# secondmind-labs/trieste

Hardware: NVIDIA H100
Metric: acquisition candidate-points/sec (EI on GPR N=4096 fp64) (higher is better)
Workload: dtype f64

## Files before the change

### trieste_b200/csrc/prescreen.cuh

```cuda
#pragma once
#include <cuda_fp16.h>
#include "kernels_f64.cuh"

namespace tb {
namespace pre {

constexpr int KS = 64;
constexpr int KH = 32;
constexpr int TH = 256;
template <int DP> struct Cpt { static constexpr int value = DP <= 12 ? 4 : DP <= 20 ? 2 : 1; };
template <int DP> struct Row { static constexpr int W = ((DP + 3 + 3) / 4) * 4; };

__host__ __device__ constexpr int tc_nk(int dp) { return (3 * dp + 2 + 15) / 16; }
__host__ __device__ constexpr int tc_mt(int dp) { return tc_nk(dp) <= 2 ? 4 : tc_nk(dp) <= 4 ? 2 : 1; }
__host__ __device__ constexpr int tc_slices(int dp) { return tc_nk(dp) <= 2 ? 16 : 8; }
__host__ __device__ constexpr int tc_slice_bytes(int dp) { return 256 * tc_nk(dp) + 32; }
__host__ __device__ constexpr int tc_cands(int dp) { return 16 * tc_mt(dp) * (TH / 32); }

struct Bound {
  double rel;
  double lin;
  double lin_max;
  double abs;
  double safety;
  double x2max;
  double mean_const;
  double pre;
};

__device__ __forceinline__ float ex2_approx(float x) {
  float y;
  asm("ex2.approx.ftz.f32 %0, %1;" : "=f"(y) : "f"(x));
  return y;
}
__device__ __forceinline__ float rsqrt_approx(float x) {
  float y;
  asm("rsqrt.approx.ftz.f32 %0, %1;" : "=f"(y) : "f"(x));
  return y;
}

template <int KIND>
__device__ __forceinline__ float kfun(float q) {
  constexpr float LN2 = 0.693147180559945309f, LN2SQ3 = 0.160151031252949358f;
  if (KIND == TB_RBF) return ex2_approx(-q);
  q = fmaxf(q, 1e-30f);
  const float s = q * rsqrt_approx(q);
  const float e = ex2_approx(-s);
  if (KIND == TB_MATERN12) return e;
  if (KIND == TB_MATERN32) return fmaf(s, LN2, 1.0f) * e;
  return fmaf(q, LN2SQ3, fmaf(s, LN2, 1.0f)) * e;
}

__device__ __forceinline__ void bound_out(const Bound& b, int64_t t, double lg, double mu, double s, int acq, double param,
                                          double var_ub, double* __restrict__ out0, double* __restrict__ out1, double& bv,
                                          int64_t& bi) {
  double e = b.safety * (fma(b.rel + lg, s, b.abs));
  const double mt = b.mean_const + mu;
  if (!(lg <= b.lin_max) || !(e <= DBL_MAX)) e = NAN;
  if (acq < 0) {
    out0[t] = mt - e;
    out1[t] = mt + e;
  } else {
    out0[t] = acq_value(acq, param, 0.0, mt - e, var_ub);
    const double v = acq_value(acq, param, 0.0, mt, var_ub);
    if (v == v) best_merge(bv, bi, v, t);
  }
}

template <int KIND, int DP>
__global__ void __launch_bounds__(TH, 2)
mean_bounds_kernel(const float* __restrict__ rows, int nst, const double* __restrict__ Xc, const double* __restrict__ inv_ls,
                   const double* __restrict__ centre, int D, int64_t M, const __grid_constant__ Bound b, int acq, double param,
                   double var_ub, double* __restrict__ out0, double* __restrict__ out1, double* __restrict__ blk_best,
                   int64_t* __restrict__ blk_idx) {
  constexpr int CPT = Cpt<DP>::value, W = Row<DP>::W, CH = KS * W / 4;
  constexpr bool EXPAND = KIND != TB_MATERN12;
  __shared__ __align__(16) float rs[2][KS * W];
  const int64_t t0 = (int64_t)blockIdx.x * (TH * CPT) + threadIdx.x;
  float xc[CPT][DP], xc2[CPT];
#pragma unroll
  for (int c = 0; c < CPT; ++c) {
    const int64_t t = t0 + (int64_t)c * TH;
    xc2[c] = 0.0f;
#pragma unroll
    for (int d = 0; d < DP; ++d) {
      xc[c][d] = (t < M && d < D) ? (float)((Xc[t * D + d] * inv_ls[d] - centre[d]) * b.pre) : 0.0f;
      xc2[c] = fmaf(xc[c][d], xc[c][d], xc2[c]);
    }
  }
  auto stage_load = [&](int kc, int buf) {
    const float* src = rows + (int64_t)kc * KS * W;
#pragma unroll
    for (int i = 0; i < (CH + TH - 1) / TH; ++i) {
      const int e = i * TH + (int)threadIdx.x;
      if (e < CH) asm volatile("cp.async.cg.shared.global [%0], [%1], 16;" ::"r"(smem_u32(&rs[buf][4 * e])), "l"(src + 4 * e) : "memory");
    }
    asm volatile("cp.async.commit_group;" ::: "memory");
  };
  double mu_d[CPT], s_d[CPT];
#pragma unroll
  for (int c = 0; c < CPT; ++c) mu_d[c] = s_d[c] = 0.0;
  stage_load(0, 0);
  for (int kc = 0; kc < nst; ++kc) {
    const int buf = kc & 1;
    if (kc + 1 < nst) {
      stage_load(kc + 1, buf ^ 1);
      asm volatile("cp.async.wait_group 1;" ::: "memory");
    } else {
      asm volatile("cp.async.wait_group 0;" ::: "memory");
    }
    __syncthreads();
#pragma unroll
    for (int h = 0; h < KS / KH; ++h) {
      float mu[CPT], sa[CPT];
#pragma unroll
      for (int c = 0; c < CPT; ++c) mu[c] = sa[c] = 0.0f;
#pragma unroll 4
      for (int j = h * KH; j < (h + 1) * KH; ++j) {
        float xr[W];
#pragma unroll
        for (int i = 0; i < W; i += 4) {
          const float4 v = *reinterpret_cast<const float4*>(&rs[buf][j * W + i]);
          xr[i] = v.x, xr[i + 1] = v.y, xr[i + 2] = v.z, xr[i + 3] = v.w;
        }
#pragma unroll
        for (int c = 0; c < CPT; ++c) {
          float q;
          if (EXPAND) {
            float dot = 0.0f;
#pragma unroll
            for (int d = 0; d < DP; ++d) dot = fmaf(xc[c][d], xr[d], dot);
            q = fmaf(-2.0f, dot, xc2[c] + xr[DP]);
          } else {
            q = 0.0f;
#pragma unroll
            for (int d = 0; d < DP; ++d) {
              const float df = xc[c][d] - xr[d];
              q = fmaf(df, df, q);
            }
          }
          const float f = kfun<KIND>(q);
          mu[c] = fmaf(xr[DP + 1], f, mu[c]);
          sa[c] = fmaf(xr[DP + 2], f, sa[c]);
        }
      }
#pragma unroll
      for (int c = 0; c < CPT; ++c) {
        mu_d[c] += (double)mu[c];
        s_d[c] += (double)sa[c];
      }
    }
    __syncthreads();
  }
  double bv = -INFINITY;
  int64_t bi = INT64_MAX;
#pragma unroll
  for (int c = 0; c < CPT; ++c) {
    const int64_t t = t0 + (int64_t)c * TH;
    if (t >= M) continue;
    const double x2 = (double)xc2[c];
    const double lg = EXPAND ? b.lin * (x2 + b.x2max) : b.lin * (sqrt(x2) + sqrt(b.x2max));
    bound_out(b, t, lg, mu_d[c], s_d[c], acq, param, var_ub, out0, out1, bv, bi);
  }
  if (acq >= 0) block_best_store(bv, bi, blk_best, blk_idx);
}

__device__ __forceinline__ void mma_f16(float (&c)[4], const uint32_t (&a)[4], uint32_t b0, uint32_t b1) {
  asm("mma.sync.aligned.m16n8k16.row.col.f32.f16.f16.f32 {%0,%1,%2,%3}, {%4,%5,%6,%7}, {%8,%9}, {%0,%1,%2,%3};"
      : "+f"(c[0]), "+f"(c[1]), "+f"(c[2]), "+f"(c[3])
      : "r"(a[0]), "r"(a[1]), "r"(a[2]), "r"(a[3]), "r"(b0), "r"(b1));
}

template <int KIND, int DP>
__global__ void __launch_bounds__(TH, 2)
tc_mean_bounds_kernel(const unsigned char* __restrict__ cols, int nsl, int npos_sl, const double* __restrict__ Xc,
                      const double* __restrict__ inv_ls, const double* __restrict__ centre, int D, int64_t M,
                      const __grid_constant__ Bound b, int acq, double param, double var_ub, double* __restrict__ out0,
                      double* __restrict__ out1, double* __restrict__ blk_best, int64_t* __restrict__ blk_idx) {
  constexpr int NK = tc_nk(DP), K = 16 * NK, MT = tc_mt(DP), SL = tc_slices(DP), SLB = tc_slice_bytes(DP);
  constexpr int CB = tc_cands(DP), STB = SL * SLB;
  constexpr int CAND_BYTES = CB * (2 * K + 4), SMEM = CAND_BYTES > 2 * STB ? CAND_BYTES : 2 * STB;
  static_assert(KIND != TB_MATERN12 && STB % 16 == 0 && SMEM <= 48 * 1024, "tc_mean_bounds_kernel geometry");
  __shared__ __align__(16) unsigned char sm[SMEM];
  const int64_t c0 = (int64_t)blockIdx.x * CB;
  {
    __half* sa = reinterpret_cast<__half*>(sm);
    float* sx2 = reinterpret_cast<float*>(sm + CB * 2 * K);
    for (int c = threadIdx.x; c < CB; c += TH) {
      const int64_t t = c0 + c;
      __half* row = sa + c * K;
      float x2 = 0.0f;
#pragma unroll
      for (int d = 0; d < DP; ++d) {
        const float x = (t < M && d < D) ? (float)((Xc[t * D + d] * inv_ls[d] - centre[d]) * b.pre) : 0.0f;
        x2 = fmaf(x, x, x2);
        const __half hi = __float2half_rn(x);
        row[d] = row[2 * DP + d] = hi;
        row[DP + d] = __float2half_rn(x - __half2float(hi));
      }
      row[3 * DP] = row[3 * DP + 1] = __float2half_rn(1.0f);
#pragma unroll
      for (int k = 3 * DP + 2; k < K; ++k) row[k] = __float2half_rn(0.0f);
      sx2[c] = x2;
    }
  }
  __syncthreads();
  const int warp = threadIdx.x >> 5, lane = threadIdx.x & 31, g = lane >> 2, tg = lane & 3;
  uint32_t af[MT][NK][4];
  float cx[MT][2];
#pragma unroll
  for (int m = 0; m < MT; ++m) {
    const int r = (warp * MT + m) * 16 + g;
    const __half* sa = reinterpret_cast<const __half*>(sm);
#pragma unroll
    for (int kk = 0; kk < NK; ++kk) {
      const __half* p = sa + r * K + kk * 16 + 2 * tg;
      af[m][kk][0] = *reinterpret_cast<const uint32_t*>(p);
      af[m][kk][1] = *reinterpret_cast<const uint32_t*>(p + 8 * K);
      af[m][kk][2] = *reinterpret_cast<const uint32_t*>(p + 8);
      af[m][kk][3] = *reinterpret_cast<const uint32_t*>(p + 8 * K + 8);
    }
    const float* sx2 = reinterpret_cast<const float*>(sm + CB * 2 * K);
    cx[m][0] = sx2[r];
    cx[m][1] = sx2[r + 8];
  }
  __syncthreads();

  auto stage_load = [&](int kc, int buf) {
    const unsigned char* src = cols + (int64_t)kc * STB;
#pragma unroll
    for (int i = 0; i < (STB / 16 + TH - 1) / TH; ++i) {
      const int e = i * TH + (int)threadIdx.x;
      if (e < STB / 16) asm volatile("cp.async.cg.shared.global [%0], [%1], 16;" ::"r"(smem_u32(sm + buf * STB + 16 * e)), "l"(src + 16 * e) : "memory");
    }
    asm volatile("cp.async.commit_group;" ::: "memory");
  };
  auto slice = [&](const unsigned char* sp, float (&acc)[MT][2]) {
    uint32_t bf[NK][2];
    if constexpr (NK % 2 == 0) {
#pragma unroll
      for (int kk = 0; kk < NK; kk += 2) {
        const uint4 v = reinterpret_cast<const uint4*>(sp)[(lane * NK + kk) / 2];
        bf[kk][0] = v.x, bf[kk][1] = v.y, bf[kk + 1][0] = v.z, bf[kk + 1][1] = v.w;
      }
    } else {
#pragma unroll
      for (int kk = 0; kk < NK; ++kk) {
        const uint2 v = reinterpret_cast<const uint2*>(sp)[lane * NK + kk];
        bf[kk][0] = v.x, bf[kk][1] = v.y;
      }
    }
    const float2 w = reinterpret_cast<const float2*>(sp + 256 * NK)[tg];
#pragma unroll
    for (int m = 0; m < MT; ++m) {
      float c[4] = {cx[m][0], cx[m][0], cx[m][1], cx[m][1]};
#pragma unroll
      for (int kk = 0; kk < NK; ++kk) mma_f16(c, af[m][kk], bf[kk][0], bf[kk][1]);
#pragma unroll
      for (int i = 0; i < 4; ++i) {
        acc[m][i >> 1] = fmaf(i & 1 ? w.y : w.x, kfun<KIND>(c[i]), acc[m][i >> 1]);
      }
    }
  };

  double pd[MT][2], qd[MT][2];
#pragma unroll
  for (int m = 0; m < MT; ++m) pd[m][0] = pd[m][1] = qd[m][0] = qd[m][1] = 0.0;
  const int nst = (nsl + SL - 1) / SL;
  stage_load(0, 0);
  for (int kc = 0; kc < nst; ++kc) {
    const int buf = kc & 1;
    if (kc + 1 < nst) {
      stage_load(kc + 1, buf ^ 1);
      asm volatile("cp.async.wait_group 1;" ::: "memory");
    } else {
      asm volatile("cp.async.wait_group 0;" ::: "memory");
    }
    __syncthreads();
    const unsigned char* st = sm + buf * STB;
    const int s0 = kc * SL, pe = min(SL, nsl - s0), bnd = min(max(npos_sl - s0, 0), pe);
    auto run = [&](int sa, int sb, double (&dd)[MT][2]) {
      float acc[MT][2];
#pragma unroll
      for (int m = 0; m < MT; ++m) acc[m][0] = acc[m][1] = 0.0f;
#pragma unroll 1
      for (int s = sa; s < sb; ++s) slice(st + s * SLB, acc);
#pragma unroll
      for (int m = 0; m < MT; ++m) dd[m][0] += (double)acc[m][0], dd[m][1] += (double)acc[m][1];
    };
    run(0, bnd, pd);
    run(bnd, pe, qd);
    __syncthreads();
  }
  double bv = -INFINITY;
  int64_t bi = INT64_MAX;
#pragma unroll
  for (int m = 0; m < MT; ++m)
#pragma unroll
    for (int h = 0; h < 2; ++h) {
      pd[m][h] += __shfl_xor_sync(0xffffffffu, pd[m][h], 1);
      qd[m][h] += __shfl_xor_sync(0xffffffffu, qd[m][h], 1);
      pd[m][h] += __shfl_xor_sync(0xffffffffu, pd[m][h], 2);
      qd[m][h] += __shfl_xor_sync(0xffffffffu, qd[m][h], 2);
      const int64_t t = c0 + (warp * MT + m) * 16 + g + 8 * h;
      if ((2 * m + h) % 4 != tg || t >= M) continue;
      const double x2 = (double)cx[m][h];
      const double lg = x2 < 0x1p28 ? b.lin * (x2 + b.x2max) : NAN;
      bound_out(b, t, lg, pd[m][h] - qd[m][h], pd[m][h] + qd[m][h], acq, param, var_ub, out0, out1, bv, bi);
    }
  if (acq >= 0) block_best_store(bv, bi, blk_best, blk_idx);
}

__global__ void probe_kernel(const double* __restrict__ Xc, int D, const int64_t* __restrict__ probe, double* __restrict__ xsel,
                             int64_t* __restrict__ isel) {
  int64_t p = *probe;
  if (p == INT64_MAX) p = 0;
  for (int d = threadIdx.x; d < D; d += blockDim.x) xsel[d] = Xc[p * D + d];
  if (threadIdx.x == 0) isel[0] = p;
}

__global__ void __launch_bounds__(256)
compact_kernel(const double* __restrict__ Xc, const double* __restrict__ ub, int64_t M, int64_t split, int D, double var_ub,
               int acq, const double* __restrict__ run_best, int64_t cap, unsigned long long* __restrict__ count,
               double* __restrict__ xsel, int64_t* __restrict__ isel) {
  const int64_t t = (int64_t)blockIdx.x * blockDim.x + threadIdx.x;
  const double thr = screen_threshold(acq, *run_best, var_ub);
  const bool keep = t < M && !(ub[t] < thr);
  const bool back = t >= split;
  const unsigned ball = __ballot_sync(0xffffffffu, keep);
  if (ball == 0u) return;
  const int lane = threadIdx.x & 31;
  const unsigned bb = __ballot_sync(0xffffffffu, keep && back), bf = ball & ~bb;
  unsigned long long base_f = 0, base_b = 0;
  if (lane == 0) {
    if (bf) base_f = atomicAdd(&count[0], (unsigned long long)__popc(bf));
    if (bb) base_b = atomicAdd(&count[1], (unsigned long long)__popc(bb));
  }
  base_f = __shfl_sync(0xffffffffu, base_f, 0);
  base_b = __shfl_sync(0xffffffffu, base_b, 0);
  if (!keep) return;
  const unsigned below = (1u << lane) - 1u;
  const int64_t r = back ? (int64_t)(base_b + (unsigned long long)__popc(bb & below)) : (int64_t)(base_f + (unsigned long long)__popc(bf & below));
  if (r >= cap) return;
  const int64_t pos = back ? cap - 1 - r : r;
  for (int d = 0; d < D; ++d) xsel[pos * D + d] = Xc[t * D + d];
  isel[pos] = t;
}

}
}
```

### trieste_b200/csrc/tb_api.cu

```cuda
#include "gp_handle.cuh"
#include "kernels_extra.cuh"
#include "prescreen.cuh"
#include "batch_ei.cuh"
#include "ehvi.cuh"
#include "int8_engines.h"
#include <chrono>
#include "factor.cuh"
#include "lbfgs.cuh"

using namespace tb;
namespace tb {
int kernels_init();
}

namespace tb {

__global__ void scale_inputs_kernel(const double* __restrict__ X, const double* __restrict__ inv_ls,
                                    int64_t N, int D, int DP, int64_t rows, double* __restrict__ Xs) {
  int64_t i = (int64_t)blockIdx.x * blockDim.x + threadIdx.x;
  if (i >= rows * DP) return;
  int64_t k = i / DP;
  int d = (int)(i % DP);
  Xs[i] = (k < N && d < D) ? X[k * D + d] * inv_ls[d] : 0.0;
}
// ... 587 lines not shown
  gp->nkc = (int)((N + BK - 1) / BK);
  gp->NB = (int)((N + BM - 1) / BM);
  gp->cache_valid = false;
  const int64_t rows = (int64_t)gp->NB * BM;
  TB_TRY(scale_inputs(gp));
  TB_TRY(gp->dAlpha.reserve(sizeof(double) * rows));
  TB_TRY(gp->sA.reserve(sizeof(double) * (3 * cap_rows * APPEND_MAX + 2 * APPEND_MAX * APPEND_MAX)));
  double* W = gp->sA.as<double>();
  double* Y = W + N * m;
  double* U = Y + N * m;
  double* S = U + N * m;
  double* R = S + m * m;
  TB_TRY(gp->dInfo.reserve(sizeof(int)));
  TB_CUDA(cudaMemsetAsync(gp->dInfo.p, 0, sizeof(int), st));
  {
    dim3 grid((unsigned)((N + 127) / 128), (unsigned)m);
    const double* Xs = gp->dXs.as<double>();
    with_kind(gp->kernel, [&](auto K) {
      append_cross_kernel<decltype(K)::value><<<grid, 128, 0, st>>>(Xs, DP, N0, N, gp->variance, gp->noise, W);
    });
    TB_LAUNCHED();
  }
  double* L = gp->dL.as<double>();
  double* Linv = gp->dLinv.as<double>();
  trmv_lower_cols_kernel<<<dim3((unsigned)((N0 + 127) / 128), (unsigned)m), 128, 0, st>>>(Linv, N0, N, W, N, Y, N);
  TB_LAUNCHED();
  append_schur_kernel<<<dim3((unsigned)m, (unsigned)m), 256, 0, st>>>(Y, W, N0, N, (int)m, S);
  TB_LAUNCHED();
  append_chol_kernel<<<1, APPEND_MAX, 0, st>>>(S, (int)m, N0, N, L, Linv, R, gp->dInfo.as<int>());
  TB_LAUNCHED();
  trmv_lower_t_cols_kernel<<<dim3((unsigned)((N0 + 7) / 8), (unsigned)m), 256, 0, st>>>(Linv, N0, N, Y, N, U, N);
  TB_LAUNCHED();
  append_rows_kernel<<<dim3((unsigned)((N0 + 127) / 128), (unsigned)m), 128, 0, st>>>(Y, U, R, (int)m, N0, N, L, Linv);
  TB_LAUNCHED();
  int info = 0;
  TB_CUDA(cudaMemcpyAsync(&info, gp->dInfo.p, sizeof(int), cudaMemcpyDeviceToHost, st));
  TB_CUDA(cudaStreamSynchronize(st));
  TB_CUDA(cudaGetLastError());
  TB_CHECK_CODE(info == 0, "tb_gp_append_data: Cholesky decomposition was not successful "
                      "(K + noise*I not positive definite at leading minor " + std::to_string(info) + ")", tb::ERR_NUMERIC);
  TB_TRY(alpha_from_linv(gp));
  return finish_cache(gp, N0);
}

int tb_gp_get_cholesky(tb_gp* gp, void* L_user) {
  TB_CHECK(gp && L_user, "tb_gp_get_cholesky: null argument");
  TB_CHECK(gp->cache_valid, "tb_gp_get_cholesky: posterior cache is not built");
  const int64_t N = gp->N;
  tb::DtypeBridge br(gp);
  double* L_out;
  TB_TRY(br.out(L_user, N * N, &L_out));
  TB_CUDA(cudaSetDevice(gp->device));
  TB_TRY(gp->sMisc.reserve(sizeof(double) * N * N));
  dim3 grid((unsigned)((N + 127) / 128), (unsigned)N);
  colmajor_lower_to_rowmajor_kernel<<<grid, 128, 0, gp->stream>>>(gp->dL.as<double>(), N, gp->sMisc.as<double>());
  TB_LAUNCHED();
  TB_CUDA(cudaMemcpyAsync(L_out, gp->sMisc.p, sizeof(double) * N * N, cudaMemcpyDefault, gp->stream));
  TB_CUDA(cudaStreamSynchronize(gp->stream));
  return br.finish();
}

}

namespace tb {

struct EvalRequest {
  int acq = -1;
  double param = 0.0;
  const double* Xc = nullptr;
  int64_t M = 0;
  double* out_vals = nullptr;
  double* out_mean = nullptr;
  double* out_var = nullptr;
  double* out_grad = nullptr;
  bool want_argmax = false;
  bool pen = false;
  double best_value = 0.0;
  int64_t best_index = -1;
};

static int launch_kstar(tb_gp* gp, const double* Xc_dev, int64_t mc, int tiles, double* KsP, double* mean) {
  const double* Xs = gp->dXs.as<double>();
  const double* al = gp->dAlpha.as<double>();
  const double* il = gp->dInvLs.as<double>();
  const int N = (int)gp->N, nkc = gp->nkc, D = gp->D;
  const double var = gp->variance, mc0 = gp->mean_const;
  cudaStream_t st = gp->stream;
  with_kind_dp(gp->kernel, gp->DP, [&](auto K, auto P) {
    kstar_panels_kernel<decltype(K)::value, decltype(P)::value><<<tiles, 512, 0, st>>>(Xs, al, Xc_dev, il, N, nkc, D, mc, 0, var, mc0,
                                                                                        KsP, mean);
  });
  TB_LAUNCHED();
  TB_CUDA(cudaGetLastError());
  return 0;
}

static int64_t chunk_tiles(const tb_gp* gp) {
  const size_t per_tile = (size_t)gp->nkc * PANEL * sizeof(double);
  const size_t budget = (size_t)1536 << 20;
  int64_t t = (int64_t)(budget / per_tile);
  t = std::max<int64_t>(t, 1);
  if (t >= NUM_SMS) t = (t / NUM_SMS) * NUM_SMS;
  return std::min<int64_t>(t, NUM_SMS * 16);
}

int kernels_init() {
  TB_CUDA(cudaFuncSetAttribute(fac::chol_diag_kernel, cudaFuncAttributeMaxDynamicSharedMemorySize, (int)(sizeof(double) * fac::FB * (fac::FB + 1))));
  TB_CUDA(cudaFuncSetAttribute(fac::chol_panel_kernel, cudaFuncAttributeMaxDynamicSharedMemorySize, (int)fac::GEMM_SMEM));
  TB_CUDA(cudaFuncSetAttribute(fac::chol_syrk_kernel, cudaFuncAttributeMaxDynamicSharedMemorySize, (int)fac::GEMM_SMEM));
  TB_CUDA(cudaFuncSetAttribute(fac::trinv_level_kernel<1>, cudaFuncAttributeMaxDynamicSharedMemorySize, (int)fac::GEMM_SMEM));
  TB_CUDA(cudaFuncSetAttribute(fac::trinv_level_kernel<2>, cudaFuncAttributeMaxDynamicSharedMemorySize, (int)fac::GEMM_SMEM));
  TB_CUDA(cudaFuncSetAttribute(fac::kinv_kernel, cudaFuncAttributeMaxDynamicSharedMemorySize, (int)fac::GEMM_SMEM));
  TB_TRY(int8_init());
  TB_CUDA(cudaFuncSetAttribute(trigemm_kernel<false, EPI_SUMSQ>, cudaFuncAttributeMaxDynamicSharedMemorySize, (int)TG_SMEM));
  TB_CUDA(cudaFuncSetAttribute(trigemm_kernel<false, EPI_SUMSQ_PACKED>, cudaFuncAttributeMaxDynamicSharedMemorySize, (int)TG_SMEM));
  TB_CUDA(cudaFuncSetAttribute(trigemm_kernel<false, EPI_PLAIN>, cudaFuncAttributeMaxDynamicSharedMemorySize, (int)TG_SMEM));
  TB_CUDA(cudaFuncSetAttribute(trigemm_kernel<true, EPI_PLAIN>, cudaFuncAttributeMaxDynamicSharedMemorySize, (int)TG_SMEM));
  return 0;
}

static int ensure_upper_panels(tb_gp* gp) {
  if (gp->upper_gen == gp->cache_gen) return 0;
  const int nkB = gp->NB * (BM / BK);
  const int64_t np = upper_panel_count(gp->NB, nkB);
  TB_TRY(gp->dLinvTP.reserve(sizeof(double) * np * PANEL));
  dim3 grid((unsigned)nkB, (unsigned)gp->NB);
  pack_upper_panels_kernel<<<grid, 256, 0, gp->stream>>>(gp->dLinv.as<double>(), gp->N, gp->NB, nkB,
                                                         gp->dLinvTP.as<double>());
  TB_LAUNCHED();
  TB_CUDA(cudaGetLastError());
  gp->upper_gen = gp->cache_gen;
  return 0;
}

static int launch_grad(tb_gp* gp, const double* xc, int64_t mc, double* grad_dev) {
  const bool wide = mc <= 2048;
  const int blocks = wide ? (int)mc : (int)((mc + 7) / 8);
  const double* Xs = gp->dXs.as<double>();
  const double* al = gp->dAlpha.as<double>();
  const double* il = gp->dInvLs.as<double>();
  const double* V = gp->sV.as<double>();
  const int64_t ldv = (int64_t)gp->NB * BM;
  const double* cmu = gp->sMisc.as<double>();
  const double* cvar = cmu + mc;
  with_kind_dp(gp->kernel, gp->DP, [&](auto K, auto P) {
    constexpr int KIND = decltype(K)::value, DP = decltype(P)::value;
    if (wide)
      grad_kernel<KIND, DP, 8><<<blocks, 256, 0, gp->stream>>>(Xs, al, xc, il, (int)gp->N, gp->D, mc, V, ldv, cmu, cvar, gp->variance,
                                                               fm::Consts(), grad_dev);
    else
      grad_kernel<KIND, DP, 1><<<blocks, 256, 0, gp->stream>>>(Xs, al, xc, il, (int)gp->N, gp->D, mc, V, ldv, cmu, cvar, gp->variance,
                                                               fm::Consts(), grad_dev);
  });
  TB_LAUNCHED();
  TB_CUDA(cudaGetLastError());
  return 0;
}

static inline bool gibbon_repulsion_kind(int acq) { return acq == TB_ACQ_GIBBON_REPULSION || acq == TB_ACQ_GIBBON; }

static int launch_gibbon_cross(tb_gp* gp, cudaStream_t st, const double* xc, int64_t mc, bool keep_u) {
  TB_TRY(gp->sGib.reserve(sizeof(double) * (size_t)mc * (2 + (keep_u ? gp->gibMp : 0))));
  double* uu = gp->sGib.as<double>();
  double* U = keep_u ? uu + 2 * mc : nullptr;
  const unsigned blocks = (unsigned)((mc + 127) / 128);
  with_kind_dp(gp->kernel, gp->DP, [&](auto K, auto P) {
    gibbon_cross_kernel<decltype(K)::value, decltype(P)::value><<<blocks, 128, 0, st>>>(
        gp->dXs.as<double>(), gp->dGibWhat.as<double>(), gp->dGibPs.as<double>(), gp->dGibLinv.as<double>(), xc, gp->dInvLs.as<double>(),
        (int)gp->N, gp->D, gp->gibM, gp->gibMp, mc, gp->variance, fm::Consts(), uu, U);
  });
  TB_LAUNCHED();
  TB_CUDA(cudaGetLastError());
  return 0;
}

static int launch_gibbon_grad(tb_gp* gp, cudaStream_t st, const double* xc, int64_t mc, double* gd) {
  const double* uu = gp->sGib.as<double>();
  const unsigned blocks = (unsigned)((mc + 7) / 8);
  with_kind_dp(gp->kernel, gp->DP, [&](auto K, auto P) {
    gibbon_grad_kernel<decltype(K)::value, decltype(P)::value><<<blocks, 256, 0, st>>>(
        gp->dXs.as<double>(), gp->dGibWhat.as<double>(), gp->dGibPs.as<double>(), gp->dGibLinv.as<double>(), xc, gp->dInvLs.as<double>(),
        (int)gp->N, gp->D, gp->gibM, gp->gibMp, mc, gp->variance, uu + 2 * mc, uu + mc, gd);
  });
  TB_LAUNCHED();
  TB_CUDA(cudaGetLastError());
  return 0;
}

static int launch_partials(tb_gp* gp, cudaStream_t st, int acq, double param, const double* partial, int G, int64_t McPad,
                           const double* mean, const double* xc, int64_t mc) {
  double* cmu = gp->sMisc.as<double>();
  const bool gib = gibbon_repulsion_kind(acq);
  if (gib) TB_TRY(launch_gibbon_cross(gp, st, xc, mc, true));
  double* g = gib ? gp->sGib.as<double>() : nullptr;
  acq_partials_kernel<<<(unsigned)((mc + 255) / 256), 256, 0, st>>>(partial, G, McPad, mean, mc, gp->variance, acq, param,
                                                                    gp->noise, gp->dMes.as<double>(), gp->mesS, cmu, cmu + mc,
                                                                    g, gp->gibW, g ? g + mc : nullptr);
  TB_LAUNCHED();
  return 0;
}

static int launch_tail(tb_gp* gp, cudaStream_t st, const EvalRequest& rq, const double* partial, int G, int64_t McPad,
                       const double* mean, int64_t mc, int64_t c0, double* d_vals, double* d_mean, double* d_var,
                       const double* xc, double* gd, const int64_t* idx_map = nullptr) {
  const int blocks = (int)((mc + 255) / 256);
  double* bb = rq.want_argmax ? gp->sBlkBest.as<double>() : nullptr;
  int64_t* bi = rq.want_argmax ? gp->sBlkIdx.as<int64_t>() : nullptr;
  TailPenalty pen;
  if (gibbon_repulsion_kind(rq.acq)) {
    if (gd)
      TB_TRY(launch_gibbon_grad(gp, st, xc, mc, gd));
    else
      TB_TRY(launch_gibbon_cross(gp, st, xc, mc, false));
    pen.gib_uu = gp->sGib.as<double>();
    pen.gib_w = gp->gibW;
  }
  if (rq.pen) {
    pen.xc = xc;
    pen.pend = gp->dPen.as<double>();
    pen.radius = pen.pend + (int64_t)gp->penP * gp->D;
    pen.scale = pen.radius + gp->penP;
    pen.grad = gd;
    pen.P = gp->penP;
    pen.D = gp->D;
    pen.kind = gp->penKind;
    tail_kernel<true><<<blocks, 256, 0, st>>>(partial, G, McPad, mean, mc, c0, gp->variance, rq.acq, rq.param, gp->noise,
                                              gp->dMes.as<double>(), gp->mesS, d_vals, d_mean, d_var, bb, bi, idx_map, pen);
  } else {
    tail_kernel<false><<<blocks, 256, 0, st>>>(partial, G, McPad, mean, mc, c0, gp->variance, rq.acq, rq.param, gp->noise,
                                               gp->dMes.as<double>(), gp->mesS, d_vals, d_mean, d_var, bb, bi, idx_map, pen);
  }
  TB_LAUNCHED();
  return 0;
}

static int ensure_kinv_dense(tb_gp* gp) {
  const int64_t N = gp->N;
  if (gp->kinv_gen == gp->cache_gen) return 0;
  cudaStream_t st = gp->stream;
  TB_TRY(gp->dKinv.reserve(sizeof(double) * N * N));
  if (gp->factor_own) {
    const unsigned t = (unsigned)((N + fac::FB - 1) / fac::FB);
    fac::kinv_kernel<<<dim3(t, t), fac::THREADS, fac::GEMM_SMEM, st>>>(gp->dLinv.as<double>(), gp->dKinv.as<double>(), N);
    TB_LAUNCHED();
  } else {
    TB_TRY(ensure_library_handles(gp));
    TB_CUDA(cudaMemcpyAsync(gp->dKinv.p, gp->dL.p, sizeof(double) * N * N, cudaMemcpyDeviceToDevice, st));
    int lwork = 0;
    cusolverStatus_t cs = cusolverDnDpotri_bufferSize(gp->cusolver, CUBLAS_FILL_MODE_LOWER, (int)N, gp->dKinv.as<double>(), (int)N, &lwork);
    TB_CHECK_CODE(cs == CUSOLVER_STATUS_SUCCESS, "cusolverDnDpotri_bufferSize failed", tb::ERR_RUNTIME);
    TB_TRY(gp->dWork.reserve(sizeof(double) * (size_t)std::max(lwork, 1)));
    cs = cusolverDnDpotri(gp->cusolver, CUBLAS_FILL_MODE_LOWER, (int)N, gp->dKinv.as<double>(), (int)N, gp->dWork.as<double>(), lwork,
                          gp->dInfo.as<int>());
    TB_CHECK_CODE(cs == CUSOLVER_STATUS_SUCCESS, "cusolverDnDpotri failed", tb::ERR_RUNTIME);
  }
  gp->kinv_gen = gp->cache_gen;
  return 0;
}

constexpr int64_t SCREEN_MIN_M = 16384;
static bool argmax_screen_wanted(const EvalRequest& rq, bool xc_dev) {
  if (!rq.want_argmax || rq.out_vals || rq.out_mean || rq.out_var || rq.out_grad || rq.pen || !xc_dev) return false;
  if (rq.acq != TB_ACQ_EI && rq.acq != TB_ACQ_LOG_EI) return false;
  if (const char* e = std::getenv("TB_ARGMAX_SCREEN"))
    if (*e) return std::atoi(e) != 0;
  return rq.M >= SCREEN_MIN_M;
}

static std::vector<unsigned char> prescreen_tc_columns(const std::vector<float>& h, int64_t N, int DP, int W, int* nsl,
                                                       int* npos_sl, bool* f16_ok) {
  const int NK = pre::tc_nk(DP), K = 16 * NK, SL = pre::tc_slices(DP), SLB = pre::tc_slice_bytes(DP);
  std::vector<int64_t> cls[2];
  for (int64_t j = 0; j < N; ++j) cls[h[(size_t)j * W + DP + 1] > 0.0f ? 0 : 1].push_back(j);
  *npos_sl = (int)((cls[0].size() + 7) / 8);
  *nsl = *npos_sl + (int)((cls[1].size() + 7) / 8);
  std::vector<unsigned char> out((size_t)((*nsl + SL - 1) / SL) * SL * SLB, 0);
  std::vector<__half> col((size_t)K);
  *f16_ok = true;
  auto split = [](float x, __half* lo) {
    const __half hi = __float2half_rn(x);
    *lo = __float2half_rn(x - __half2float(hi));
    return hi;
  };
  for (int c = 0; c < 8 * *nsl; ++c) {
    const int k = c < 8 * *npos_sl ? 0 : 1;
    const int64_t i = k == 0 ? c : c - 8 * *npos_sl;
    if (i >= (int64_t)cls[k].size()) continue;
    const float* r = &h[(size_t)cls[k][i] * W];
    std::fill(col.begin(), col.end(), __float2half_rn(0.0f));
    for (int d = 0; d < DP; ++d) {
      __half lo;
      const __half hi = split(r[d], &lo);
      col[d] = col[DP + d] = __float2half_rn(-2.0f * __half2float(hi));
      col[2 * DP + d] = __float2half_rn(-2.0f * __half2float(lo));
      *f16_ok = *f16_ok && std::fabs(r[d]) < 16384.0f;
    }
    col[3 * DP] = split(r[DP], &col[3 * DP + 1]);
    *f16_ok = *f16_ok && r[DP] < 32768.0f;
    unsigned char* sp = &out[(size_t)(c / 8) * SLB];
    const int g = c % 8;
    for (int tg = 0; tg < 4; ++tg)
      for (int kk = 0; kk < NK; ++kk)
        for (int hf = 0; hf < 2; ++hf) std::memcpy(sp + ((g * 4 + tg) * NK + kk) * 8 + 4 * hf, &col[kk * 16 + 8 * hf + 2 * tg], 4);
    std::memcpy(sp + 256 * NK + 4 * g, &r[DP + 2], 4);
  }
  return out;
}

static int prescreen_ensure(tb_gp* gp) {
  if (gp->pre_gen == gp->cache_gen) return 0;
  const int64_t N = gp->N;
  const int D = gp->D, DP = gp->DP;
  const int W = ((DP + 3 + 3) / 4) * 4;
  const int64_t rows = ((N + pre::KS - 1) / pre::KS) * pre::KS;
  cudaStream_t st = gp->stream;
  std::vector<double> xs((size_t)N * DP), al((size_t)N);
  TB_CUDA(cudaMemcpyAsync(xs.data(), gp->dXs.p, sizeof(double) * N * DP, cudaMemcpyDeviceToHost, st));
  TB_CUDA(cudaMemcpyAsync(al.data(), gp->dAlpha.p, sizeof(double) * N, cudaMemcpyDeviceToHost, st));
  TB_CUDA(cudaStreamSynchronize(st));
  const double LOG2E = 1.4426950408889634, LN2 = 0.6931471805599453;
  double pre2, cq;
  switch (gp->kernel) {
    case TB_RBF: pre2 = 0.5 * LOG2E, cq = LN2; break;
    case TB_MATERN12: pre2 = LOG2E * LOG2E, cq = 0.0; break;
    case TB_MATERN32: pre2 = 3.0 * LOG2E * LOG2E, cq = 0.5 * LN2 * LN2; break;
    default: pre2 = 5.0 * LOG2E * LOG2E, cq = LN2 * LN2 / 6.0; break;
  }
  const double pre = std::sqrt(pre2);
  std::vector<double> centre((size_t)DP, 0.0), half_width((size_t)DP, 0.0);
  double unc2 = 0.0;
  for (int d = 0; d < D; ++d) {
    double lo = INFINITY, hi = -INFINITY;
    for (int64_t j = 0; j < N; ++j) lo = std::min(lo, xs[j * DP + d]), hi = std::max(hi, xs[j * DP + d]);
    centre[d] = 0.5 * (lo + hi);
    half_width[d] = 0.5 * (hi - lo);
  }
  std::vector<float> h((size_t)rows * W, 0.0f);
  double x2max = 0.0, asum = 0.0, c2 = 0.0, box2 = 0.0;
  for (int d = 0; d < D; ++d) {
    c2 += centre[d] * centre[d];
    const double hw = half_width[d] * pre;
    box2 += hw * hw;
  }
  for (int64_t j = 0; j < N; ++j) {
    float* r = &h[(size_t)j * W];
    double n2 = 0.0, u2 = 0.0;
    for (int d = 0; d < D; ++d) {
      r[d] = (float)((xs[j * DP + d] - centre[d]) * pre);
      n2 += (double)r[d] * (double)r[d];
      u2 += xs[j * DP + d] * xs[j * DP + d];
    }
    r[DP] = (float)n2;
    const float a = (float)(gp->variance * al[j]);
    r[DP + 1] = a;
    r[DP + 2] = std::fabs(a);
    x2max = std::max(x2max, (double)r[DP]);
    unc2 = std::max(unc2, u2);
    asum += std::fabs((double)a);
  }
  const double u = std::ldexp(1.0, -24), mufu = std::ldexp(1.0, -21);
  const bool expand = gp->kernel != TB_MATERN12;
  double kappa = 0.0, s0 = 0.0, tail = 0.0;
  if (gp->kernel != TB_RBF) {
    kappa = 1.01 * (mufu + u + (expand ? 0.0 : (2 * DP + 2) * u / 2));
    auto T = [&](double s) {
      const double p = gp->kernel == TB_MATERN12 ? 1.0 : gp->kernel == TB_MATERN32 ? 1.0 + s : 1.0 + s + s * s / 3.0;
      return s * p * std::exp(-s);
    };
    double best = INFINITY;
    for (double s = 4.0; s <= 48.0; s += 1.0) {
      const double cost = s * 0.01 * asum + T(s) * asum;
      if (cost < best) best = cost, s0 = s;
    }
    tail = T(s0);
  }
  double rel = mufu + 4 * u
               + 32 * u / (1 - 32 * u)
               + kappa * s0
               + (double)(N + 64) * std::ldexp(1.0, -52)
               + 1e-15;
  const double lin_max = std::ldexp(1.0, -10);
  double lin;
  std::vector<unsigned char> tc;
  double terms = (double)rows;
  gp->pre_tc = false;
  if (expand) {
    const double l64 = cq * (2 * DP + 10) * std::ldexp(1.0, -52);
    rel += l64 * pre2 * (c2 + unc2);
    lin = cq * (2 * DP + 10) * u + l64;
    const double rd = std::sqrt((double)DP);
    const double lin_q = (4 + 1.01 * DP + 1) * u
                         + 4.01 * std::ldexp(1.0, -22)
                         + 1.01 * rd * std::ldexp(1.0, -25)
                         + pre::tc_nk(DP) * 2.01 * 24 * std::ldexp(1.0, -23);
    const double abs_q = 1.01 * rd * std::ldexp(1.0, -24) + std::ldexp(1.0, -25);
    const double lin_tc = cq * lin_q + l64;
    bool f16_ok = false;
    if (1.01 * lin_tc * (box2 + 1.01 * x2max) <= 0.5 * lin_max) {
      tc = prescreen_tc_columns(h, N, DP, W, &gp->pre_nsl, &gp->pre_npos_sl, &f16_ok);
      gp->pre_tc = f16_ok;
    }
    if (gp->pre_tc) {
      terms = 8.0 * gp->pre_nsl;
      lin = lin_tc;
      rel += cq * abs_q;
    }
  } else {
    lin = LN2 * u;
  }
  gp->pre_rel = 1.01 * rel;
  gp->pre_lin = 1.01 * lin;
  gp->pre_lin_max = lin_max;
  gp->pre_abs = 1.01 * (asum * (2700.0 * std::ldexp(1.0, -126) + kappa * tail) + 2.0 * terms * std::ldexp(1.0, -149));
  gp->pre_scale = pre;
  gp->pre_x2max = 1.01 * x2max;
  const size_t bytes = gp->pre_tc ? tc.size() : sizeof(float) * h.size();
  TB_TRY(gp->dPreRows.reserve(bytes));
  TB_TRY(gp->dPreCentre.reserve(sizeof(double) * DP));
  TB_CUDA(cudaMemcpyAsync(gp->dPreRows.p, gp->pre_tc ? (const void*)tc.data() : (const void*)h.data(), bytes, cudaMemcpyHostToDevice, st));
  TB_CUDA(cudaMemcpyAsync(gp->dPreCentre.p, centre.data(), sizeof(double) * DP, cudaMemcpyHostToDevice, st));
  TB_CUDA(cudaStreamSynchronize(st));
  gp->pre_gen = gp->cache_gen;
  return 0;
}

static int prescreen_blocks(const tb_gp* gp, int64_t M) {
  const int DP = gp->DP;
  const int64_t per = gp->pre_tc ? pre::tc_cands(DP) : (int64_t)pre::TH * (DP <= 12 ? 4 : DP <= 20 ? 2 : 1);
  return (int)((M + per - 1) / per);
}

static int launch_mean_bounds(tb_gp* gp, cudaStream_t st, const double* Xc, int64_t M, int acq, double param, double var_ub,
                              double* out0, double* out1, double* blk_best, int64_t* blk_idx) {
  TB_TRY(prescreen_ensure(gp));
  pre::Bound b;
  b.rel = gp->pre_rel;
  b.lin = gp->pre_lin;
  b.lin_max = gp->pre_lin_max;
  b.abs = gp->pre_abs;
  b.safety = 4.0;
  b.x2max = gp->pre_x2max;
  b.mean_const = gp->mean_const;
  b.pre = gp->pre_scale;
  const int D = gp->D;
  const double* il = gp->dInvLs.as<double>();
  const double* cen = gp->dPreCentre.as<double>();
  const unsigned blocks = (unsigned)prescreen_blocks(gp, M);
  with_kind_dp(gp->kernel, gp->DP, [&](auto K, auto P) {
    constexpr int KIND = decltype(K)::value, DP = decltype(P)::value;
    if (!gp->pre_tc) {
      const int nst = (int)((gp->N + pre::KS - 1) / pre::KS);
      pre::mean_bounds_kernel<KIND, DP><<<blocks, pre::TH, 0, st>>>(gp->dPreRows.as<float>(), nst, Xc, il, cen, D, M, b, acq, param,
                                                                    var_ub, out0, out1, blk_best, blk_idx);
    } else if constexpr (KIND != TB_MATERN12) {
      pre::tc_mean_bounds_kernel<KIND, DP><<<blocks, pre::TH, 0, st>>>(gp->dPreRows.as<unsigned char>(), gp->pre_nsl, gp->pre_npos_sl,
                                                                       Xc, il, cen, D, M, b, acq, param, var_ub, out0, out1, blk_best,
                                                                       blk_idx);
    }
  });
  TB_LAUNCHED();
  TB_CUDA(cudaGetLastError());
  return 0;
}

enum class Engine {
  F64,
  OZ21,
  OZ15,
};

static int select_engine(tb_gp* gp, bool need_v, Engine* eng) {
  if (!(gp->engine == 1 && gp->N <= 16384)) {
    if (need_v) TB_TRY(ensure_upper_panels(gp));
    *eng = Engine::F64;
    return 0;
  }
  if (need_v) TB_TRY(ensure_kinv_dense(gp));
  bool single_pass;
  TB_TRY(int8_select(gp, need_v, &single_pass));
  *eng = single_pass ? Engine::OZ15 : Engine::OZ21;
  return 0;
}

static int eng_tile_width(const tb_gp* gp, Engine e) { return e == Engine::F64 ? BT : int8_tile_width(gp, e == Engine::OZ15); }
static size_t eng_tile_bytes(const tb_gp* gp, Engine e) {
  return e == Engine::F64 ? (size_t)gp->nkc * PANEL * sizeof(double) : int8_tile_bytes(gp, e == Engine::OZ15);
}

static int eng_groups(const tb_gp* gp, Engine e, int tiles) {
  const int fill = (2 * NUM_SMS + tiles - 1) / tiles;
  if (e == Engine::F64) return tiles >= NUM_SMS ? 1 : std::max(1, std::min(fill, gp->NB));
  return std::max(std::max(1, (gp->NB + 3) / 4), std::min(gp->NB, fill));
}

static int eng_kstar(tb_gp* gp, Engine e, const double* xc, int64_t mc, int tiles, const KSplit* split = nullptr, bool wide = false) {
  double* mean = gp->sMean.as<double>();
  if (e == Engine::F64) return launch_kstar(gp, xc, mc, tiles, gp->sKs.as<double>(), mean);
  return int8_kstar(gp, e == Engine::OZ15, xc, mc, tiles, gp->sKs.as<int8_t>(), mean, split, wide);
}

static int eng_variance(tb_gp* gp, Engine e, int tiles, int G, int64_t McPad, bool packed_a, int kper = 0) {
  cudaStream_t st = gp->stream;
  double* partial = gp->sPartial.as<double>();
  if (e != Engine::F64) return int8_variance(gp, e == Engine::OZ15, gp->sKs.as<int8_t>(), tiles, G, McPad, partial, kper);
  if (packed_a)
    trigemm_kernel<false, EPI_SUMSQ_PACKED><<<dim3(tiles, G), TG_THREADS, TG_SMEM, st>>>(
        gp->dLinvP.as<double>(), gp->sKs.as<double>(), gp->NB, gp->nkc, G, McPad, partial, gp->sA.as<double>(), nullptr, 0);
  else
    trigemm_kernel<false, EPI_SUMSQ><<<dim3(tiles, G), TG_THREADS, TG_SMEM, st>>>(
        gp->dLinvP.as<double>(), gp->sKs.as<double>(), gp->NB, gp->nkc, G, McPad, partial, nullptr, nullptr, 0);
  TB_LAUNCHED();
  TB_CUDA(cudaGetLastError());
  return 0;
}

static int eng_store_a(tb_gp* gp, Engine e, int tiles, int64_t McPad, double* out) {
  const int64_t lda = (int64_t)gp->NB * BM;
  const int G = eng_groups(gp, e, tiles);
  if (e != Engine::F64) return int8_store(gp, e == Engine::OZ15, false, gp->sKs.as<int8_t>(), tiles, G, McPad, out, lda);
  trigemm_kernel<false, EPI_PLAIN><<<dim3(tiles, G), TG_THREADS, TG_SMEM, gp->stream>>>(gp->dLinvP.as<double>(), gp->sKs.as<double>(),
                                                                                        gp->NB, gp->nkc, G, McPad, nullptr, nullptr, out, lda);
  TB_LAUNCHED();
  TB_CUDA(cudaGetLastError());
  return 0;
}

static int eng_store_v(tb_gp* gp, Engine e, int tiles, int64_t McPad) {
  const int64_t ldv = (int64_t)gp->NB * BM;
  double* V = gp->sV.as<double>();
  if (e == Engine::OZ21) {
    const int G = std::max(1, std::min(gp->NB, std::max((gp->NB + 7) / 8, (2 * NUM_SMS + tiles - 1) / tiles)));
    return int8_store(gp, false, true, gp->sKs.as<int8_t>(), tiles, G, McPad, V, ldv);
  }
  const int G = eng_groups(gp, e, tiles);
  if (e == Engine::OZ15) return int8_store(gp, true, true, gp->sKs.as<int8_t>(), tiles, G, McPad, V, ldv);
  trigemm_kernel<true, EPI_PLAIN><<<dim3(tiles, G), TG_THREADS, TG_SMEM, gp->stream>>>(gp->dLinvTP.as<double>(), gp->sA.as<double>(), gp->NB,
                                                                                       gp->NB * (BM / BK), G, McPad, nullptr, nullptr, V, ldv);
  TB_LAUNCHED();
  TB_CUDA(cudaGetLastError());
  return 0;
}


static int argmax_reset(tb_gp* gp) {
  const double init_v = -INFINITY;
  const int64_t init_i = INT64_MAX;
  TB_CUDA(cudaMemcpyAsync(gp->sRun.p, &init_v, 8, cudaMemcpyHostToDevice, gp->stream));
  TB_CUDA(cudaMemcpyAsync((char*)gp->sRun.p + 8, &init_i, 8, cudaMemcpyHostToDevice, gp->stream));
  return 0;
}
static int argmax_fold(tb_gp* gp, int64_t n) {
  argmax_fold_kernel<<<1, 256, 0, gp->stream>>>(gp->sBlkBest.as<double>(), gp->sBlkIdx.as<int64_t>(), (int)((n + 255) / 256),
                                                gp->sRun.as<double>(), reinterpret_cast<int64_t*>((char*)gp->sRun.p + 8));
  TB_LAUNCHED();
  return 0;
}
static int argmax_read(tb_gp* gp, EvalRequest& rq) {
  TB_CUDA(cudaMemcpyAsync(&rq.best_value, gp->sRun.p, 8, cudaMemcpyDeviceToHost, gp->stream));
  TB_CUDA(cudaMemcpyAsync(&rq.best_index, (char*)gp->sRun.p + 8, 8, cudaMemcpyDeviceToHost, gp->stream));
  return 0;
}

template <class F>
static int profiled_gemm(tb_gp* gp, double flops, F&& launch) {
  if (!gp->profile) return launch();
  cudaEvent_t e0 = nullptr, e1 = nullptr;
  TB_CUDA(cudaEventCreate(&e0));
  TB_CUDA(cudaEventCreate(&e1));
  TB_CUDA(cudaEventRecord(e0, gp->stream));
  TB_TRY(launch());
  TB_CUDA(cudaEventRecord(e1, gp->stream));
  gp->prof_events.emplace_back(e0, e1);
  gp->prof_event_flops.push_back(flops);
  return 0;
}
static int profile_fold(tb_gp* gp) {
  for (size_t i = 0; i < gp->prof_events.size(); ++i) {
    float ms = 0.f;
    TB_CUDA(cudaEventElapsedTime(&ms, gp->prof_events[i].first, gp->prof_events[i].second));
    gp->prof_ms += ms;
    gp->prof_flops += gp->prof_event_flops[i];
    gp->prof_launches += 1;
    cudaEventDestroy(gp->prof_events[i].first);
    cudaEventDestroy(gp->prof_events[i].second);
  }
  gp->prof_events.clear();
  gp->prof_event_flops.clear();
  return 0;
}

struct EvalOut {
  double *vals = nullptr, *mean = nullptr, *var = nullptr, *grad = nullptr;
};

static int eval_chunk(tb_gp* gp, const EvalRequest& rq, Engine e, const double* xc, int64_t n, int64_t c0, int G, const EvalOut& o,
                      const int64_t* idx_map = nullptr, const KSplit* split = nullptr) {
  cudaStream_t st = gp->stream;
  const int nt = eng_tile_width(gp, e);
  const int tiles = (int)((n + nt - 1) / nt);
  const int64_t McPad = (int64_t)tiles * nt;
  const double* partial = gp->sPartial.as<double>();
  const double* mean = gp->sMean.as<double>();
  const int kper = idx_map && e != Engine::F64 ? int8_split_kper(gp, e == Engine::OZ15, tiles, G) : 0;
  TB_TRY(eng_kstar(gp, e, xc, n, tiles, split, kper > 0));
  TB_TRY(profiled_gemm(gp, (double)McPad * (double)gp->N * (double)gp->N,
                       [&] { return eng_variance(gp, e, tiles, G, McPad, o.grad != nullptr, kper); }));
  if (o.grad) {
    TB_TRY(launch_partials(gp, st, rq.acq, rq.param, partial, G, McPad, mean, xc, n));
    TB_TRY(eng_store_v(gp, e, tiles, McPad));
    TB_TRY(launch_grad(gp, xc, n, o.grad));
  }
  TB_TRY(launch_tail(gp, st, rq, partial, G, McPad, mean, n, c0, o.vals, o.mean, o.var, xc, o.grad, idx_map));
  return rq.want_argmax ? argmax_fold(gp, n) : 0;
}

static int argmax_screened(tb_gp* gp, const EvalRequest& rq, Engine e, int64_t chunk_cap, int G, bool* done) {
  *done = false;
  cudaStream_t st = gp->stream;
  const int D = gp->D, nt = eng_tile_width(gp, e);
  const int64_t M = rq.M;
  const int64_t cap = std::max<int64_t>(1, M / 4);
  TB_TRY(prescreen_ensure(gp));
  const int sblocks = (int)((M + 255) / 256), bblocks = prescreen_blocks(gp, M);
  TB_TRY(gp->sScrUb.reserve(sizeof(double) * (size_t)M));
  TB_TRY(gp->sScrX.reserve(sizeof(double) * (size_t)cap * D));
  TB_TRY(gp->sScrIdx.reserve(sizeof(int64_t) * (size_t)cap));
  TB_TRY(gp->sScrBlk.reserve(16 * (size_t)bblocks + 32));
  double* ub = gp->sScrUb.as<double>();
  double* xsel = gp->sScrX.as<double>();
  int64_t* isel = gp->sScrIdx.as<int64_t>();
  double* bb = gp->sScrBlk.as<double>();
  int64_t* bi = reinterpret_cast<int64_t*>(bb + bblocks);
  double* probe_v = reinterpret_cast<double*>(bi + bblocks);
  int64_t* probe_i = reinterpret_cast<int64_t*>(probe_v + 1);
  unsigned long long* count = reinterpret_cast<unsigned long long*>(probe_v + 2);
  const int64_t split = ((M - 1) / chunk_cap) * chunk_cap;
  const KSplit ks_full = int8_kstar_split(gp, e == Engine::OZ15, (int)(chunk_cap / nt)),
               ks_last = int8_kstar_split(gp, e == Engine::OZ15, (int)((M - split + nt - 1) / nt));
  const bool same_split = ks_full.ksplit == ks_last.ksplit && ks_full.kc_per == ks_last.kc_per;
  const double var_ub = std::fmax(gp->variance, 1e-12);
  const double init_v = -INFINITY;
  const int64_t init_i = INT64_MAX;
  TB_CUDA(cudaMemcpyAsync(probe_v, &init_v, 8, cudaMemcpyHostToDevice, st));
  TB_CUDA(cudaMemcpyAsync(probe_i, &init_i, 8, cudaMemcpyHostToDevice, st));
  TB_TRY(launch_mean_bounds(gp, st, rq.Xc, M, rq.acq, rq.param, var_ub, ub, nullptr, bb, bi));
  argmax_fold_kernel<<<1, 256, 0, st>>>(bb, bi, bblocks, probe_v, probe_i);
  TB_LAUNCHED();
  pre::probe_kernel<<<1, 32, 0, st>>>(rq.Xc, D, probe_i, xsel, isel);
  TB_LAUNCHED();
  bool probe_last = true;
  if (!same_split) {
    int64_t p = 0;
    TB_CUDA(cudaMemcpyAsync(&p, probe_i, 8, cudaMemcpyDeviceToHost, st));
    TB_CUDA(cudaStreamSynchronize(st));
    probe_last = (p == INT64_MAX ? 0 : p) >= split;
  }
  const EvalOut none;
  TB_TRY(eval_chunk(gp, rq, e, xsel, 1, 0, G, none, isel, probe_last ? &ks_last : &ks_full));
  TB_CUDA(cudaMemsetAsync(count, 0, 16, st));
  pre::compact_kernel<<<sblocks, 256, 0, st>>>(rq.Xc, ub, M, split, D, var_ub, rq.acq, gp->sRun.as<double>(), cap, count, xsel, isel);
  TB_LAUNCHED();
  unsigned long long n[2] = {0, 0};
  TB_CUDA(cudaMemcpyAsync(n, count, 16, cudaMemcpyDeviceToHost, st));
  TB_CUDA(cudaStreamSynchronize(st));
  TB_CUDA(cudaGetLastError());
  if (n[0] + n[1] > (unsigned long long)cap) return argmax_reset(gp);
  const int64_t nf = (int64_t)n[0], nb = (int64_t)n[1];
  for (int64_t s0 = 0; s0 < nf; s0 += chunk_cap)
    TB_TRY(eval_chunk(gp, rq, e, xsel + s0 * D, std::min<int64_t>(chunk_cap, nf - s0), 0, G, none, isel + s0, &ks_full));
  for (int64_t s0 = cap - nb; s0 < cap; s0 += chunk_cap)
    TB_TRY(eval_chunk(gp, rq, e, xsel + s0 * D, std::min<int64_t>(chunk_cap, cap - s0), 0, G, none, isel + s0, &ks_last));
  *done = true;
  return 0;
}

struct ChunkPlan {
  int nt = BT;
  int64_t chunk_cap = 0;
  int G = 0;
};
static ChunkPlan plan_chunks(const tb_gp* gp, Engine e, bool grad, int64_t M) {
  ChunkPlan p;
  p.nt = eng_tile_width(gp, e);
  const size_t budget = (size_t)1280 << 20;
  int64_t max_tiles;
  if (e != Engine::F64 && !grad) {
    max_tiles = std::max<int64_t>(1, (int64_t)(budget / eng_tile_bytes(gp, e)));
    if (max_tiles >= 2 * NUM_SMS) max_tiles = (max_tiles / (2 * NUM_SMS)) * (2 * NUM_SMS);
    else if (max_tiles >= NUM_SMS) max_tiles = NUM_SMS;
    max_tiles = std::min<int64_t>(max_tiles, 8 * NUM_SMS);
  } else if (e == Engine::OZ15) {
    const size_t v_bytes = (size_t)p.nt * gp->NB * BM * sizeof(double);
    max_tiles = std::max<int64_t>(1, (int64_t)(budget / std::max(eng_tile_bytes(gp, e), v_bytes)));
    if (max_tiles >= NUM_SMS) max_tiles = (max_tiles / NUM_SMS) * NUM_SMS;
  } else {
    max_tiles = chunk_tiles(gp);
  }
  p.chunk_cap = std::min<int64_t>(max_tiles * p.nt, ((M + p.nt - 1) / p.nt) * p.nt);
  if (e != Engine::F64 && !grad) p.G = eng_groups(gp, e, (int)(p.chunk_cap / p.nt));
  return p;
}

static int check_eval(const tb_gp* gp, const EvalRequest& rq) {
  TB_CHECK(gp->cache_valid, "posterior cache is not built: call tb_gp_update_posterior_cache first");
  TB_CHECK(rq.M >= 0, "negative candidate count");
  if (rq.want_argmax) TB_CHECK(rq.M > 0, "argmax over an empty candidate set");
  return 0;
}
// ... 1718 lines not shown
```

Measured before the change: 321.1 million.

## Fold Matern polynomial weights into slice data and offload sqrt to FMA Newton

The tensor-core prescreen slices now hold precomputed per-column weights w, w·ln2 and w·ln2²/3, so the Matern polynomial factor becomes a couple of FMAs using these weights. The kernel replaces the rsqrt-based sqrt with sqrt.approx on most slots, and on three of every eight slots it uses a bit-trick Newton sqrt that runs on the FMA pipe. This spreads transcendental work between the SFU and FMA units. The error bound is widened to cover the Newton sqrt's relative error, and each slice grows by 64 bytes, which adds shared-memory and load traffic.

```diff
diff --git a/trieste_b200/csrc/prescreen.cuh b/trieste_b200/csrc/prescreen.cuh
--- a/trieste_b200/csrc/prescreen.cuh
+++ b/trieste_b200/csrc/prescreen.cuh
@@ -14,8 +14,11 @@
 __host__ __device__ constexpr int tc_nk(int dp) { return (3 * dp + 2 + 15) / 16; }
 __host__ __device__ constexpr int tc_mt(int dp) { return tc_nk(dp) <= 2 ? 4 : tc_nk(dp) <= 4 ? 2 : 1; }
 __host__ __device__ constexpr int tc_slices(int dp) { return tc_nk(dp) <= 2 ? 16 : 8; }
-__host__ __device__ constexpr int tc_slice_bytes(int dp) { return 256 * tc_nk(dp) + 32; }
+__host__ __device__ constexpr int tc_slice_bytes(int dp) { return 256 * tc_nk(dp) + 96; }
 __host__ __device__ constexpr int tc_cands(int dp) { return 16 * tc_mt(dp) * (TH / 32); }
+constexpr int TC_NEWTON_EIGHTHS = 3;
+__host__ __device__ constexpr bool tc_newton_slot(int v) { return (v * TC_NEWTON_EIGHTHS) % 8 < TC_NEWTON_EIGHTHS; }
+constexpr double TC_NEWTON_REL = 4.52e-7;
 
 struct Bound {
   double rel;
@@ -49,6 +52,28 @@
   if (KIND == TB_MATERN12) return e;
   if (KIND == TB_MATERN32) return fmaf(s, LN2, 1.0f) * e;
   return fmaf(q, LN2SQ3, fmaf(s, LN2, 1.0f)) * e;
+}
+
+__device__ __forceinline__ float sqrt_approx(float x) {
+  float y;
+  asm("sqrt.approx.ftz.f32 %0, %1;" : "=f"(y) : "f"(x));
+  return y;
+}
+__device__ __forceinline__ float sqrt_newton(float x) {
+  float y = __uint_as_float(0x5f1ffff9u - (__float_as_uint(x) >> 1));
+  y *= fmaf(-0.703952253f, (x * y) * y, 1.68191409f);
+  const float s = x * y;
+  return s * fmaf(-0.500000179f, s * y, 1.50000048f);
+}
+
+template <int KIND, bool NEWTON>
+__device__ __forceinline__ float tc_term(float q, float w, float wl, float wl3, float acc) {
+  if (KIND == TB_RBF) return fmaf(w, ex2_approx(-q), acc);
+  const float x = fabsf(q);
+  const float s = NEWTON ? sqrt_newton(x) : sqrt_approx(x);
+  const float e = ex2_approx(-s);
+  const float t = KIND == TB_MATERN32 ? fmaf(wl, s, w) : fmaf(wl3, x, fmaf(wl, s, w));
+  return fmaf(t, e, acc);
 }
 
 __device__ __forceinline__ void bound_out(const Bound& b, int64_t t, double lg, double mu, double s, int acq, double param,
@@ -250,7 +275,8 @@
         bf[kk][0] = v.x, bf[kk][1] = v.y;
       }
     }
-    const float2 w = reinterpret_cast<const float2*>(sp + 256 * NK)[tg];
+    const float4 w = reinterpret_cast<const float4*>(sp + 256 * NK)[tg];
+    const float2 w3 = reinterpret_cast<const float2*>(sp + 256 * NK + 64)[tg];
 #pragma unroll
     for (int m = 0; m < MT; ++m) {
       float c[4] = {cx[m][0], cx[m][0], cx[m][1], cx[m][1]};
@@ -258,7 +284,9 @@
       for (int kk = 0; kk < NK; ++kk) mma_f16(c, af[m][kk], bf[kk][0], bf[kk][1]);
 #pragma unroll
       for (int i = 0; i < 4; ++i) {
-        acc[m][i >> 1] = fmaf(i & 1 ? w.y : w.x, kfun<KIND>(c[i]), acc[m][i >> 1]);
+        const float wi = i & 1 ? w.y : w.x, wl = i & 1 ? w.w : w.z, wl3 = i & 1 ? w3.y : w3.x;
+        float& a = acc[m][i >> 1];
+        a = tc_newton_slot(4 * m + i) ? tc_term<KIND, true>(c[i], wi, wl, wl3, a) : tc_term<KIND, false>(c[i], wi, wl, wl3, a);
       }
     }
   };
diff --git a/trieste_b200/csrc/tb_api.cu b/trieste_b200/csrc/tb_api.cu
--- a/trieste_b200/csrc/tb_api.cu
+++ b/trieste_b200/csrc/tb_api.cu
@@ -913,7 +913,12 @@
     for (int tg = 0; tg < 4; ++tg)
       for (int kk = 0; kk < NK; ++kk)
         for (int hf = 0; hf < 2; ++hf) std::memcpy(sp + ((g * 4 + tg) * NK + kk) * 8 + 4 * hf, &col[kk * 16 + 8 * hf + 2 * tg], 4);
-    std::memcpy(sp + 256 * NK + 4 * g, &r[DP + 2], 4);
+    const double LN2 = 0.6931471805599453;
+    const float w[3] = {r[DP + 2], (float)((double)r[DP + 2] * LN2), (float)((double)r[DP + 2] * (LN2 * LN2 / 3.0))};
+    unsigned char* wp = sp + 256 * NK;
+    std::memcpy(wp + 16 * (g / 2) + 4 * (g % 2), &w[0], 4);
+    std::memcpy(wp + 16 * (g / 2) + 8 + 4 * (g % 2), &w[1], 4);
+    std::memcpy(wp + 64 + 4 * g, &w[2], 4);
   }
   return out;
 }
@@ -1014,7 +1019,12 @@
     if (gp->pre_tc) {
       terms = 8.0 * gp->pre_nsl;
       lin = lin_tc;
-      rel += cq * abs_q;
+      rel += cq * abs_q + u;
+      if (kappa > 0.0) {
+        const double kappa_tc = 1.01 * std::max(mufu, pre::TC_NEWTON_REL);
+        rel += (kappa_tc - kappa) * s0;
+        kappa = kappa_tc;
+      }
     }
   } else {
     lin = LN2 * u;
```

New measurement: 334.3 million, median of 6. 1.04x the previous value.
